# ANSSI-FR/libecc

Hardware: AMD Instinct MI355X
Metric: scalar-mults/sec (secp256r1, batch=2^20, variable base, affine out, bit-exact vs CPU) (higher is better)
Workload: dtype u32 (29-bit limbs, v_mad_u64_u32 integer MAD, u64 accumulators)

## Files before the change

libecc_amd/build.py:

```python
import os
import subprocess
import sys

HERE = os.path.dirname(os.path.abspath(__file__))
CSRC = os.path.join(HERE, "csrc")
LIBDIR = os.path.join(HERE, "lib")
LIB = os.path.join(LIBDIR, "libecc_amd.so")
SOURCES = ["ecamd_kernels.hip", "ecamd_p256_kernel.hip", "ecamd_hash.hip", "ecamd_host.cpp", "ecamd_multi.cpp"]
DEPS = ["ecamd_madchain.h", "ecamd_field.h", "ecamd_point.h", "ecamd_u29.h", "ecamd_p256.h", "ecamd_u29g.h", "ecamd_jacg.h",
        "ecamd_internal.h", "ecamd_lattice.h", "ecamd_randmod.h", "ecamd_recover.h", "ecamd_recover_kernels.h",
        "ecamd_sigfam.h", "ecamd_sigfam_kernels.h", "ecamd_sighash.h", "ecamd_sighash_kernels.h",
        "ecamd_curve_table.inc"]
HOST_DEPS = [os.path.join("..", "..", "include", "libecc_amd.h")]
HIPCC = os.environ.get("HIPCC", "/opt/rocm/bin/hipcc")
FLAGS = ["--offload-arch=gfx950", "-O3", "-std=c++17", "-fPIC", "-Wall", "-Wno-unused-function",
         "-Wno-bitwise-instead-of-logical", "-DU29_ASM_MAD"]


def _stale(target, inputs):
    if not os.path.exists(target):
        return True
    t = os.path.getmtime(target)
    return any(os.path.getmtime(i) > t for i in inputs)


G29_SIZES = [192, 224, 255, 256, 320, 384, 448, 511, 512, 521]


def _jobs():
    jobs = [(src, os.path.splitext(src)[0] + ".o", []) for src in SOURCES]
    jobs += [("ecamd_g29_kernel.hip", f"ecamd_g29_{pb}.o", [f"-DG29_PB={pb}"] + (["-DG29_WAVES=2"] if pb in (511, 512, 521) else []))
             for pb in G29_SIZES]
    jobs.append(("ecamd_g29_kernel.hip", "ecamd_g29_521m.o", ["-DG29_PB=521", "-DG29_M521P", "-DG29_WAVES=2"]))
    jobs.append(("ecamd_g29_kernel.hip", "ecamd_g29_255c.o", ["-DG29_PB=255", "-DG29_P25519", "-DG29_WAVES=3"]))
    jobs.append(("ecamd_g29_kernel.hip", "ecamd_g29_256k.o", ["-DG29_PB=256", "-DG29_K256", "-DG29_WAVES=3"]))
    jobs.append(("ecamd_g29_kernel.hip", "ecamd_g29_448g.o", ["-DG29_PB=448", "-DG29_P448"]))
    jobs.append(("ecamd_g29_kernel.hip", "ecamd_g29_384n.o", ["-DG29_PB=384", "-DG29_P384S"]))
    jobs.append(("ecamd_g29_kernel.hip", "ecamd_g29_224s.o", ["-DG29_PB=224", "-DG29_P224S"]))
    jobs.append(("ecamd_g29_kernel.hip", "ecamd_g29_192s.o", ["-DG29_PB=192", "-DG29_P192S"]))
    jobs.append(("ecamd_g29_kernel.hip", "ecamd_g29_dispatch.o", ["-DG29_DISPATCH"]))
    return jobs


def build(force=False, verbose=False):
    from concurrent.futures import ThreadPoolExecutor
    os.makedirs(LIBDIR, exist_ok=True)
    deps = [os.path.join(CSRC, d) for d in DEPS]
    hdeps = [os.path.join(CSRC, d) for d in HOST_DEPS]
    todo, objs = [], []
    for src, obj, extra in _jobs():
        spath, opath = os.path.join(CSRC, src), os.path.join(LIBDIR, obj)
        objs.append(opath)
        cmd = [HIPCC] + FLAGS + extra + ["-x", "hip", "-c", spath, "-o", opath]
        try:
            same_cmd = open(opath + ".cmd").read() == " ".join(cmd)
        except OSError:
            same_cmd = False
        if force or not same_cmd or _stale(opath, [spath] + deps + (hdeps if src.endswith(".cpp") else [])):
            todo.append(cmd)

    def run(cmd):
        if verbose:
            print(" ".join(cmd))
        subprocess.check_call(cmd)
        if "-c" in cmd:
            with open(cmd[-1] + ".cmd", "w") as f:
                f.write(" ".join(cmd))

    with ThreadPoolExecutor(max_workers=max(1, min(8, os.cpu_count() or 1))) as ex:
        list(ex.map(run, todo))
    if force or _stale(LIB, objs):
        run([HIPCC, "--offload-arch=gfx950", "-shared", "-fPIC", "-o", LIB] + objs + ["-ldl", "-lpthread"])
    return LIB


if __name__ == "__main__":
    print(build(force="--force" in sys.argv, verbose=True))
```

libecc_amd/csrc/ecamd_host.cpp:

```cpp
#include <hip/hip_runtime.h>
#include <stdint.h>
#include <string.h>
#include <strings.h>
#include <stdio.h>
#include <stdlib.h>
#include <string>
#include <vector>
#include <functional>
#include <mutex>
#include <sys/random.h>

#include "../../include/libecc_amd.h"
#include "ecamd_internal.h"
#include "ecamd_sighash.h"

static thread_local std::string g_err;
static int fail(const std::string &m)
{
	g_err = m;
	return -1;
}
#define HIPCHK(expr) \
	do { \
		hipError_t e_ = (expr); \
// ... 103 lines not shown
	big_trim(r);
	return r;
}
static Big big_mod(const Big &a, const Big &m)
{
	Big r(1, 0);
	for (int bit = big_bitlen(a) - 1; bit >= 0; bit--) {
		Big t(r.size() + 1, 0);
		for (size_t i = 0; i < r.size(); i++) {
			t[i] |= r[i] << 1;
			t[i + 1] |= r[i] >> 31;
		}
		t[0] |= (a[(size_t)bit / 32] >> (bit % 32)) & 1u;
		big_trim(t);
		r = (big_cmp(t, m) >= 0) ? big_sub(t, m) : t;
	}
	return r;
}
static Big big_pow2(int e)
{
	Big r((size_t)e / 32 + 1, 0);
	r[(size_t)e / 32] = 1u << (e % 32);
	return r;
}
static Big big_mulmod(const Big &a, const Big &b, const Big &m) { return big_mod(big_mul(a, b), m); }
static Big big_powmod(const Big &a, const Big &e, const Big &m)
{
	Big r(1, 1), base = big_mod(a, m);
	for (int i = big_bitlen(e) - 1; i >= 0; i--) {
		r = big_mulmod(r, r, m);
		if ((e[(size_t)i / 32] >> (i % 32)) & 1u) {
			r = big_mulmod(r, base, m);
		}
	}
	return r;
}
static void big_store(uint32_t *dst, int nw, const Big &a)
{
	for (int i = 0; i < nw; i++) {
		dst[i] = (size_t)i < a.size() ? a[(size_t)i] : 0;
	}
}
static void big_to_be(uint8_t *dst, int len, const Big &a)
{
	for (int i = 0; i < len; i++) {
		int pos = len - 1 - i;
		dst[i] = ((size_t)pos / 4 < a.size()) ? (uint8_t)(a[(size_t)pos / 4] >> (8 * (pos % 4))) : 0;
	}
}

struct CurveRow {
	const char *name;
	int type;
	const char *p, *a, *b, *order, *gx, *gy, *q, *h;
};
static const CurveRow g_curve_rows[] = {
#include "ecamd_curve_table.inc"
};

#define ECAMD_NSTAGE 30
struct ecamd_ctx {
	int device;
	hipStream_t stream;
	uint32_t max_chunk;
	uint32_t *tbl;
	size_t tbl_bytes;
	uint32_t *tbl_fast;
	size_t tbl_fast_bytes;
	uint8_t *prep_scratch;
	size_t prep_scratch_bytes;
	uint8_t *stage[ECAMD_NSTAGE];
	size_t stage_bytes[ECAMD_NSTAGE];
	hipEvent_t busy;
	hipStream_t last_stream;
	bool inflight;
	hipStream_t copy_stream;
	hipEvent_t in_ready[2];
	hipStream_t side_stream;
	hipEvent_t side_fork, side_done, side_mid, side_aux;
	hipEvent_t side_hi, side_red;
	hipStream_t side2_stream;
	hipEvent_t side2_fork, side2_done;
	bool side2_ok;
	bool side_ok;
	uint32_t host_chunk;
	uint32_t host_first_min;
	ecamd_host_ready_fn ready_fn = nullptr;
	void *ready_arg = nullptr;
	uint8_t *hbuf[2][6];
	size_t hbuf_bytes[2][6];
	uint32_t comb_min_batch;
	bool secret_scalars;
	int eddsa_msm;
	uint32_t msm_min, msm_k;
	uint8_t *msm;
	size_t msm_bytes;
	uint8_t msm_seed_bytes[32];
	bool msm_seed_valid;
	bool timing;
	hipEvent_t ev[ECAMD_NTIMED + 1];
	bool ev_valid;
	hipEvent_t ev_dom[2];
	bool ev_dom_valid;
	std::mutex mu;
};

struct ecamd_curve {
	ecamd_ctx *ctx;
	int nw;
	int slot;
	int qslot;
	int curve_type;
	int qnw;
	int clen;
	int qlen;
	int pbits, qbits;
	Big p, a, b, order, gx, gy, q;
	uint8_t *d_gen;
	uint32_t cofactor;
	int ed_state;
	const char *ed_err;
	EcamdEdDecodeArgs ed_tmpl;
	uint32_t ed_cof_dbl;
	int ed448_state;
	const char *ed448_err;
	EcamdEd448DecodeArgs ed448_tmpl;
	uint8_t ed448_c4[56];
	uint32_t ed_2d[9];
	uint32_t ed_Bx[9], ed_By[9];
	int xdh_state;
	const char *xdh_err;
	EcamdXdhPrepArgs xdh_tmpl;
	uint32_t xdh_A3[17];
	uint8_t xdh_cof;
	int sqrt_state;
	EcamdYfromXArgs sqrt_tmpl;
	bool is_p256;
	int gslot;
	int gpslot;
	int gqslot;
	int gflavour;
	uint32_t *d_comb4;
	bool comb4_off;
	uint32_t *d_gtab;
	uint32_t *d_comb;
	bool comb_off;
	uint32_t *d_edcomb;
	bool edcomb_off;
	uint32_t qdig[9];
};

static const int k_widths[] = {6, 7, 8, 10, 12, 14, 16, 17};

static int pick_nw(int pbits)
{
	for (int w : k_widths) {
		if (32 * w >= pbits) {
			return w;
		}
	}
	return 0;
}

extern "C" int ecamd_device_count(void)
{
	int n = 0;
// ... 27 lines not shown
		if (getenv("ECAMD_NO_COMB") != nullptr) {
			c->comb_min_batch = 0;
		}
	}
	c->tbl = nullptr;
	c->tbl_bytes = 0;
	c->tbl_fast = nullptr;
	c->tbl_fast_bytes = 0;
	for (int i = 0; i < ECAMD_NSTAGE; i++) {
		c->stage[i] = nullptr;
		c->stage_bytes[i] = 0;
	}
	c->prep_scratch = nullptr;
	c->prep_scratch_bytes = 0;
	c->last_stream = nullptr;
	c->inflight = false;
	if (hipEventCreateWithFlags(&c->busy, hipEventDisableTiming) != hipSuccess) {
		delete c;
		return fail("ecamd_ctx_create: hipEventCreate failed");
	}
	c->timing = false;
	c->secret_scalars = false;
	c->eddsa_msm = 1;
	c->msm_min = 1u << 17;
	c->msm_k = 0;
	{
		const char *e = getenv("ECAMD_MSM_MIN");
		if (e) {
			c->msm_min = (uint32_t)strtoul(e, nullptr, 10);
		}
		e = getenv("ECAMD_MSM_K");
		if (e) {
			c->msm_k = (uint32_t)strtoul(e, nullptr, 10);
		}
	}
	c->msm = nullptr;
	c->msm_bytes = 0;
	c->msm_seed_valid = false;
	c->ev_valid = false;
	c->ev_dom_valid = false;
	for (int i = 0; i <= ECAMD_NTIMED; i++) {
		if (hipEventCreate(&c->ev[i]) != hipSuccess) {
			delete c;
			return fail("ecamd_ctx_create: hipEventCreate failed");
		}
	}
	if (hipEventCreate(&c->ev_dom[0]) != hipSuccess || hipEventCreate(&c->ev_dom[1]) != hipSuccess) {
		delete c;
		return fail("ecamd_ctx_create: hipEventCreate failed");
	}
	memset(c->hbuf, 0, sizeof(c->hbuf));
	memset(c->hbuf_bytes, 0, sizeof(c->hbuf_bytes));
	{
		const char *e = getenv("ECAMD_HOST_CHUNK");
		c->host_chunk = e ? (uint32_t)strtoul(e, nullptr, 10) : (1u << 19);
		if (c->host_chunk == 0) {
			c->host_chunk = 1u << 19;
		}
		e = getenv("ECAMD_HOST_RAMP_MIN");
		c->host_first_min = e ? (uint32_t)strtoul(e, nullptr, 10) : (1u << 16);
		if (c->host_first_min == 0) {
			c->host_first_min = 1u << 16;
		}
	}
	if (hipStreamCreateWithFlags(&c->copy_stream, hipStreamNonBlocking) != hipSuccess ||
	    hipEventCreateWithFlags(&c->in_ready[0], hipEventDisableTiming) != hipSuccess ||
	    hipEventCreateWithFlags(&c->in_ready[1], hipEventDisableTiming) != hipSuccess) {
		delete c;
		return fail("ecamd_ctx_create: copy stream creation failed");
	}
	if (hipStreamCreateWithFlags(&c->stream, hipStreamNonBlocking) != hipSuccess) {
		delete c;
		return fail("ecamd_ctx_create: hipStreamCreate failed");
	}
	if (hipStreamCreateWithFlags(&c->side_stream, hipStreamNonBlocking) != hipSuccess ||
	    hipEventCreateWithFlags(&c->side_fork, hipEventDisableTiming) != hipSuccess ||
	    hipEventCreateWithFlags(&c->side_done, hipEventDisableTiming) != hipSuccess ||
	    hipEventCreateWithFlags(&c->side_mid, hipEventDisableTiming) != hipSuccess ||
	    hipEventCreateWithFlags(&c->side_aux, hipEventDisableTiming) != hipSuccess ||
	    hipEventCreateWithFlags(&c->side_hi, hipEventDisableTiming) != hipSuccess ||
	    hipEventCreateWithFlags(&c->side_red, hipEventDisableTiming) != hipSuccess ||
	    hipStreamCreateWithFlags(&c->side2_stream, hipStreamNonBlocking) != hipSuccess ||
	    hipEventCreateWithFlags(&c->side2_fork, hipEventDisableTiming) != hipSuccess ||
	    hipEventCreateWithFlags(&c->side2_done, hipEventDisableTiming) != hipSuccess) {
		delete c;
		return fail("ecamd_ctx_create: side stream creation failed");
	}
	c->side_ok = getenv("ECAMD_NO_SIDE_STREAM") == nullptr;
	c->side2_ok = c->side_ok;
	*out = c;
	return 0;
}

extern "C" void ecamd_ctx_destroy(ecamd_ctx *c)
{
	if (!c) {
		return;
	}
	(void)hipSetDevice(c->device);
	(void)hipStreamSynchronize(c->stream);
	if (c->tbl) {
		(void)hipFree(c->tbl);
	}
	if (c->tbl_fast) {
		(void)hipFree(c->tbl_fast);
	}
	if (c->msm) {
		(void)hipFree(c->msm);
	}
	for (int i = 0; i < ECAMD_NSTAGE; i++) {
		if (c->stage[i]) {
			(void)hipFree(c->stage[i]);
		}
	}
	if (c->prep_scratch) {
		(void)hipFree(c->prep_scratch);
	}
	for (int i = 0; i <= ECAMD_NTIMED; i++) {
		(void)hipEventDestroy(c->ev[i]);
	}
	(void)hipEventDestroy(c->ev_dom[0]);
	(void)hipEventDestroy(c->ev_dom[1]);
	(void)hipStreamDestroy(c->stream);
	(void)hipStreamDestroy(c->copy_stream);
	(void)hipStreamSynchronize(c->side_stream);
	(void)hipStreamDestroy(c->side_stream);
	(void)hipEventDestroy(c->side_fork);
	(void)hipEventDestroy(c->side_done);
	(void)hipEventDestroy(c->side_mid);
	(void)hipEventDestroy(c->side_aux);
	(void)hipEventDestroy(c->side_hi);
	(void)hipEventDestroy(c->side_red);
	(void)hipStreamSynchronize(c->side2_stream);
	(void)hipStreamDestroy(c->side2_stream);
	(void)hipEventDestroy(c->side2_fork);
	(void)hipEventDestroy(c->side2_done);
	(void)hipEventDestroy(c->in_ready[0]);
	(void)hipEventDestroy(c->in_ready[1]);
	(void)hipEventDestroy(c->busy);
	for (int b = 0; b < 2; b++) {
		for (int k = 0; k < 6; k++) {
			if (c->hbuf[b][k]) {
				(void)hipFree(c->hbuf[b][k]);
			}
		}
	}
	delete c;
}

extern "C" int ecamd_ctx_set_max_chunk(ecamd_ctx *c, uint32_t max_items)
{
	if (!c || max_items == 0) {
		return fail("ecamd_ctx_set_max_chunk: bad argument");
	}
	c->max_chunk = max_items;
	return 0;
}

extern "C" int ecamd_ctx_set_eddsa_msm(ecamd_ctx *c, int mode, uint32_t min_items, uint32_t items_per_lane)
{
	if (!c || mode < 0 || mode > 2 || items_per_lane > 64) {
		return fail("ecamd_ctx_set_eddsa_msm: bad argument");
	}
	std::lock_guard<std::mutex> lk(c->mu);
	c->eddsa_msm = mode;
	if (min_items) {
		c->msm_min = min_items;
	}
	c->msm_k = items_per_lane;
	return 0;
}

extern "C" int ecamd_ctx_set_msm_seed(ecamd_ctx *c, const uint8_t seed[32])
{
	if (!c || !seed) {
		return fail("ecamd_ctx_set_msm_seed: bad argument");
	}
	std::lock_guard<std::mutex> lk(c->mu);
	memcpy(c->msm_seed_bytes, seed, 32);
	c->msm_seed_valid = true;
	return 0;
}

extern "C" int ecamd_ctx_discard_msm_seed(ecamd_ctx *c)
{
	if (!c) {
		return fail("ecamd_ctx_discard_msm_seed: NULL context");
	}
	std::lock_guard<std::mutex> lk(c->mu);
	if (c->msm_seed_valid) {
		memset(c->msm_seed_bytes, 0, sizeof(c->msm_seed_bytes));
		c->msm_seed_valid = false;
	}
	return 0;
}

extern "C" int ecamd_ctx_set_secret_scalars(ecamd_ctx *c, int on)
{
	if (!c) {
		return fail("ecamd_ctx_set_secret_scalars: NULL context");
	}
	std::lock_guard<std::mutex> lk(c->mu);
	c->secret_scalars = on != 0;
	return 0;
}

extern "C" int ecamd_ctx_enable_kernel_timing(ecamd_ctx *c, int on)
{
	if (!c) {
		return fail("ecamd_ctx_enable_kernel_timing: NULL context");
	}
	std::lock_guard<std::mutex> lk(c->mu);
	c->timing = on != 0;
	c->ev_valid = false;
	c->ev_dom_valid = false;
	return 0;
}

extern "C" int ecamd_ctx_kernel_times(ecamd_ctx *c, double *ms, int n)
// ... 907 lines not shown
	const bool secret = ctx->secret_scalars;
	const bool fast256 = cv->is_p256 && slen <= 68;
	const bool fastg = !fast256 && cv->gslot >= 0 && slen <= ecamd_g29_max_slen(cv->pbits);
	const bool comb_ok = !secret && (cv->is_p256 ? slen <= 32 : slen <= ecamd_g29_comb_max_slen(cv->pbits));
	const bool fast = !redo_only && (fast256 || fastg);
	if (fast && !d_points && comb_ok) {
		maybe_build_comb(ctx, const_cast<ecamd_curve *>(cv), n);
	}
	if (fast && fastg && !d_points && secret && n >= 64) {
		maybe_build_comb4(ctx, const_cast<ecamd_curve *>(cv));
	}
	{
		uint8_t *t = (uint8_t *)ctx->tbl;
		const int rc = ensure(&t, &ctx->tbl_bytes, tbl_bytes_for(cv, stride));
		ctx->tbl = (uint32_t *)t;
		if (rc) {
			return -1;
		}
	}
	if (fast) {
		uint8_t *t = (uint8_t *)ctx->tbl_fast;
		const size_t per_item = fast256 ? P256_SCRATCH_PER_ITEM
						: ((size_t)ecamd_g29_table_words(cv->pbits, cv->gflavour) + ecamd_g29_affine_words(cv->pbits, cv->gflavour)) * 4;
		const int rc = ensure(&t, &ctx->tbl_fast_bytes, (size_t)stride * per_item);
		ctx->tbl_fast = (uint32_t *)t;
		if (rc) {
			return -1;
		}
	}
	for (uint32_t off = 0; off < n; off += chunk) {
		const uint32_t m = (n - off) < chunk ? (n - off) : chunk;
		EcamdSmulArgs A;
		A.scalars = d_scalars + (size_t)off * sstride;
		A.sstride = sstride;
		A.pstride = d_points ? 2u * (uint32_t)cv->clen : 0u;
		A.points = d_points ? d_points + (size_t)off * 2 * cv->clen : cv->d_gen;
		A.out = d_out + (size_t)off * 2 * cv->clen;
		A.status = d_status + off;
		A.tbl = ctx->tbl;
		A.n = m;
		A.slen = slen;
		A.clen = (uint32_t)cv->clen;
		A.stride = stride;
		A.slot = cv->slot;
		A.only_redo = redo_only ? 1 : 0;
		A.lut = nullptr;
		A.lut_kind = 0;
		A.stg = nullptr;
		A.masked = secret ? 1 : 0;
		A.scalars2 = nullptr;
		A.s2len = 0;
		if (d_scalars2) {
			if (!fastg || !d_points || !cv->d_comb) {
				return fail("internal: fused double-scalar loop requested without its preconditions");
			}
			EcamdSmulArgs Fa = A;
			Fa.tbl = ctx->tbl_fast;
			Fa.stg = ctx->tbl_fast + (size_t)stride * (size_t)ecamd_g29_table_words(cv->pbits, cv->gflavour);
			Fa.lut = cv->d_comb;
			Fa.lut_kind = 2u;
			Fa.scalars2 = d_scalars2 + (size_t)off * slen;
			Fa.s2len = slen;
			Fa.masked = 0;
			hipEvent_t *ev = (ctx->timing && off == 0) ? ctx->ev : nullptr;
			HIPCHK(ecamd_launch_smul_g29(cv->pbits, cv->gslot, Fa, s, ev, cv->gflavour));
			ctx->ev_valid = ctx->ev_valid || (ev != nullptr);
			continue;
		}
		if (fast) {
			EcamdSmulArgs Fa = A;
			Fa.tbl = ctx->tbl_fast;
			Fa.stg = ctx->tbl_fast + (size_t)stride * (fast256 ? (size_t)(P256_TAB_BYTES / 4) : (size_t)ecamd_g29_table_words(cv->pbits, cv->gflavour));
			if (!d_points) {
				const bool use_comb = cv->d_comb && comb_ok;
				Fa.lut = use_comb ? cv->d_comb : (fast256 ? cv->d_gtab : nullptr);
				Fa.lut_kind = use_comb ? 1u : 0u;
				if (secret && cv->d_comb4 && (fast256 ? slen <= 32 : slen <= 4 * (uint32_t)((cv->pbits + 31) / 32))) {
					Fa.lut = cv->d_comb4;
					Fa.lut_kind = 3u;
				}
			}
			hipEvent_t *ev = (ctx->timing && off == 0) ? ctx->ev : nullptr;
			if (fast256) {
				HIPCHK(ecamd_launch_smul_p256(Fa, s, ev));
			} else {
				HIPCHK(ecamd_launch_smul_g29(cv->pbits, cv->gslot, Fa, s, ev, cv->gflavour));
			}
			ctx->ev_valid = ctx->ev_valid || (ev != nullptr);
			A.only_redo = 1;
		}
		HIPCHK(ecamd_launch_smul(cv->nw, A, s));
	}
	return 0;
}

struct HostArr {
	const uint8_t *in;
	uint8_t *out;
	size_t stride;
};

template <class Core>
static int host_pipeline(ecamd_ctx *ctx, int pbits, uint32_t n, const std::vector<HostArr> &arrs, Core core, uint32_t even_chunk = 0)
{
	const uint32_t chunk = even_chunk && even_chunk < ctx->host_chunk ? (n < even_chunk ? n : even_chunk) : (n < ctx->host_chunk ? n : ctx->host_chunk);
	const size_t na = arrs.size();
	if (na > 6) {
		return fail("internal: too many host arrays");
	}
	static const bool no_ramp = getenv("ECAMD_NO_HOST_RAMP") != nullptr;
	std::vector<uint32_t> sched;
	{
		uint32_t left = n;
		if (const char *e = getenv("ECAMD_HOST_SCHEDULE")) {
			while (*e && left) {
				uint32_t v = (uint32_t)strtoul(e, nullptr, 10);
				v = v < 1 ? 1 : (v > left ? left : v);
				sched.push_back(v);
				left -= v;
				e = strchr(e, ',');
				if (!e) {
					break;
				}
				e++;
			}
		} else if (even_chunk && n > chunk) {
			const uint32_t m = ctx->host_first_min < chunk ? ctx->host_first_min : chunk;
			if (m < chunk && left > m) {
				sched.push_back(m);
				left -= m;
			}
		} else if (n > chunk && !no_ramp && pbits <= 256) {
			for (uint32_t m = ctx->host_first_min < chunk ? ctx->host_first_min : chunk; m < chunk && left > m + m; m += m) {
				sched.push_back(m);
				left -= m;
			}
		} else if (n > chunk && !no_ramp) {
			const uint32_t m = chunk / 8 < ctx->host_first_min ? ctx->host_first_min : chunk / 8;
			if (m < chunk) {
				sched.push_back(m);
				left -= m;
			}
		}
		while (left) {
			const uint32_t m = (left <= chunk + chunk / 4) ? left : chunk;
			sched.push_back(m);
			left -= m;
		}
	}
	uint32_t largest = 0;
	for (uint32_t m : sched) {
		largest = m > largest ? m : largest;
	}
	const int nbuf = sched.size() > 1 ? 2 : 1;
	for (int b = 0; b < nbuf; b++) {
		for (size_t k = 0; k < na; k++) {
			if (ensure(&ctx->hbuf[b][k], &ctx->hbuf_bytes[b][k], (size_t)largest * arrs[k].stride)) {
				return -1;
			}
		}
	}
	hipStream_t cs = ctx->copy_stream, s = ctx->stream;
	StreamScope scope(ctx, s);
	auto copy_in = [&](uint32_t off, uint32_t m, int b) -> int {
		if (ctx->ready_fn) {
			ctx->ready_fn(ctx->ready_arg, off, m);
		}
// ... 4617 lines not shown
```

libecc_amd/csrc/ecamd_internal.h:

```cpp
#pragma once
#include <stdlib.h>
#include <hip/hip_runtime.h>
#include <stdint.h>

#define ECAMD_WINDOW 4
#define ECAMD_TBL_ENTRIES (1 << ECAMD_WINDOW)
#define ECAMD_STATUS_TAB 0xFC
#define ECAMD_STATUS_JAC 0xFD
#define ECAMD_STATUS_REDO 0xFE
#define ECAMD_MAX_SLOTS_HOST 16
#define P256_TAB_BYTES 512u
#define P256_STG_QUADS 70u

struct EcamdSmulArgs {
	const uint8_t *scalars;
	const uint8_t *points;
	uint8_t *out;
	uint8_t *status;
	uint32_t *tbl;
	uint32_t *stg;
	uint32_t n, slen, clen, pstride, stride;
	uint32_t sstride;
	int slot;
	int only_redo;
// ... 53 lines not shown
	uint8_t *result;
	uint32_t n, clen, qlen, jmax;
	uint32_t q[17];
	int slot;
	const uint8_t *only;
};
struct EcamdEcdsaSignArgs {
	const uint8_t *privs, *nonces, *digests;
	const uint8_t *kG, *stkG;
	uint8_t *sigs, *status;
	uint32_t n, clen, qlen, hlen, qbits, jmax;
	int qslot;
};
hipError_t ecamd_launch_ecdsa_sign(int nw, const EcamdEcdsaSignArgs &a, hipStream_t s);
hipError_t ecamd_launch_ecdsa_prep(int nw, const EcamdEcdsaPrepArgs &a, hipStream_t s);
hipError_t ecamd_launch_ecdsa_fin(int nw, const EcamdEcdsaFinArgs &a, hipStream_t s);

struct EcamdSigPrepArgs {
	EcamdEcdsaPrepArgs p;
	uint8_t *target;
	int alg;
};
struct EcamdSigSignArgs {
	EcamdEcdsaSignArgs a;
	int alg;
};
hipError_t ecamd_launch_sig_prep(int nw, const EcamdSigPrepArgs &a, hipStream_t s);
hipError_t ecamd_launch_sig_sign(int nw, const EcamdSigSignArgs &a, hipStream_t s);

struct EcamdRecoverPrepArgs {
	const uint8_t *sigs;
	const uint8_t *digests;
	uint8_t *u, *v;
	uint8_t *x;
	uint8_t *flags;
	uint32_t n, qlen, clen, hlen, qbits;
	int qslot;
	uint8_t p_be[72];
};
struct EcamdRecoverPointArgs {
	const uint8_t *x, *y1;
	const uint8_t *flags, *yst;
	uint8_t *R;
	uint32_t n, clen;
};
struct EcamdRecoverFinArgs {
	const uint8_t *A, *stA;
	const uint8_t *B, *stB;
	const uint8_t *flags;
	const uint8_t *yst;
	uint8_t *out1, *out2;
	uint8_t *st1, *st2;
	uint32_t n, clen;
	int slot;
};
hipError_t ecamd_launch_recover_prep(int qnw, const EcamdRecoverPrepArgs &a, hipStream_t s);
hipError_t ecamd_launch_recover_point(const EcamdRecoverPointArgs &a, hipStream_t s);
hipError_t ecamd_launch_recover_fin(int nw, const EcamdRecoverFinArgs &a, hipStream_t s);
hipError_t ecamd_launch_recover_redo(int nw, const EcamdRecoverFinArgs &a, hipStream_t s);

struct EcamdHsigArgs {
	const uint8_t *sigs;
	const uint8_t *inputs;
	const uint8_t *privs, *nonces;
	uint8_t *u, *v;
	uint8_t *flags;
	const uint8_t *W, *stW;
	uint8_t *slots;
	const uint8_t *dg;
	uint8_t *out;
	uint8_t *status;
	uint32_t n, qlen, clen, hsize, sstride;
	int qslot, alg, sign;
};
hipError_t ecamd_launch_hsig_prep(int qnw, const EcamdHsigArgs &a, hipStream_t s);
hipError_t ecamd_launch_hsig_fill(const EcamdHsigArgs &a, hipStream_t s);
hipError_t ecamd_launch_hsig_cmp(const EcamdHsigArgs &a, hipStream_t s);
hipError_t ecamd_launch_hsig_sign(int qnw, const EcamdHsigArgs &a, hipStream_t s);

int ecamd_nw_supported(int nw);
hipError_t ecamd_upload_curve(int nw, int slot, const void *curvek, size_t bytes);
hipError_t ecamd_launch_smul(int nw, const EcamdSmulArgs &a, hipStream_t s);
#define ECAMD_NTIMED 5
hipError_t ecamd_launch_smul_p256(const EcamdSmulArgs &a, hipStream_t s, hipEvent_t *ev);
hipError_t ecamd_launch_verify_p256(const EcamdSmulArgs &pubkeys, const uint8_t *u1, const uint8_t *u2, const uint8_t *sigs,
				    const uint8_t *flags, const uint32_t *gtbl, int gtbl_is_comb, const uint32_t *qdigits,
				    uint8_t *result, hipStream_t s, hipEvent_t *dom = nullptr, hipEvent_t scalars_ready = nullptr);
hipError_t ecamd_launch_comb_build_p256(const uint8_t *points, uint32_t n, uint32_t *table, hipStream_t s);
struct EcamdXdhPrepArgs {
	const uint8_t *k, *u;
	uint8_t *scalars;
	uint8_t *points;
	uint8_t *flags;
	uint32_t n, len, ebits, mode;
	uint32_t cof_dbl;
	uint32_t e[17];
	uint32_t A[17], A3[17], sm1[17];
	uint32_t g_A[16], g_A3[16], g_sm1[16];
	int slot;
};
struct EcamdXdhFinArgs {
	const uint8_t *pts;
	const uint8_t *stk;
	const uint8_t *flags;
	uint8_t *out;
	uint8_t *status;
	uint32_t n, len;
	uint32_t A3[17];
	int slot;
};
hipError_t ecamd_launch_xdh_prep(int nw, const EcamdXdhPrepArgs &a, hipStream_t s);
hipError_t ecamd_launch_xdh_fin(int nw, const EcamdXdhFinArgs &a, hipStream_t s);

struct EcamdEdDecodeArgs {
	const uint8_t *encA;
	const uint8_t *encR;
	uint32_t strideA, strideR;
	uint8_t *pointsA, *pointsR;
	uint8_t *flagsA, *flagsR;
	uint32_t n, len, cof_dbl;
	uint32_t a[17], d[17], sm1[17], alpha[17], A3[17];
	uint32_t g_d[9], g_sm1[9], g_alpha[9], g_A3[9];
	uint32_t *edA;
	uint32_t *edR;
	int slot;
};
hipError_t ecamd_launch_ed_decode_ed_c25519(const EcamdEdDecodeArgs &a, int gslot, hipStream_t s);
struct EcamdEdSmulArgs {
	const uint32_t *edA;
	const uint8_t *scalars;
	const uint8_t *flags;
	uint32_t *tbl;
	uint32_t *rec;
	uint8_t *out, *status;
	uint32_t n;
	uint32_t g_2d[9], g_alpha[9], g_A3[9];
	const uint32_t *edR;
	uint8_t *flagsR;
	uint8_t *outR;
};
#define ECAMD_EDT_ITEM_WORDS 320
#define ECAMD_EDR_REC_WORDS 28
struct EcamdEdTailConsts {
	uint32_t g_2d[9], g_alpha[9], g_A3[9];
};
#define ECAMD_EDC_ENT_WORDS 32
#define ECAMD_EDC_ENTRIES (16u * 32768u + 1u)
struct EcamdEdSmul2Args {
	const uint32_t *edA, *edR;
	const uint8_t *flagsA, *flagsR, *flagsS;
	const uint32_t *uv;
	const uint8_t *meta;
	uint32_t *tbl;
	uint32_t *rec;
	uint32_t n;
	uint32_t g_2d[9];
};
struct EcamdEdTailArgs {
	const uint32_t *rec;
	const uint32_t *edR;
	const uint8_t *flagsA, *flagsR, *flagsS;
	const uint8_t *S_be;
	const uint8_t *sp_be;
	const uint8_t *meta;
	const uint32_t *comb;
	uint8_t *result;
	uint32_t n, cof_dbl;
// ... 348 lines not shown
```

libecc_amd/csrc/ecamd_p256_kernel.hip:

```cpp
#include <hip/hip_runtime.h>
#include "ecamd_p256.h"
#include "ecamd_internal.h"

using namespace p256;

typedef uint8_t u8;

#define TBL_WORDS_PER_ENTRY 40
#define TBL_ENTRIES 8
#define TAB_ENT_WORDS 16
#define TAB_ITEM_WORDS (TBL_ENTRIES * TAB_ENT_WORDS)
#define STG_ENT_QUADS 10
#define STG_ITEM_QUADS (7 * STG_ENT_QUADS)
static_assert(TAB_ITEM_WORDS * 4 <= P256_TAB_BYTES && STG_ITEM_QUADS <= P256_STG_QUADS, "scratch exceeds the host's per-item sizing");
#ifndef FIN_K
#define FIN_K 8
#endif
#ifndef AFF_K
#define AFF_K 8
#endif
static inline int p256_items_per_inversion(uint32_t n, int kmax)
{
	const int k = n >= (1u << 19) ? 8 : (n >= (1u << 17) ? 4 : 2);
	return k < kmax ? k : kmax;
}

static __device__ __forceinline__ void load_be256(const u8 *src, u32 *w)
{
	if ((((uintptr_t)src) & 15) == 0) {
		const uint4 a = *(const uint4 *)src, b = *(const uint4 *)(src + 16);
		w[7] = __builtin_bswap32(a.x);
		w[6] = __builtin_bswap32(a.y);
		w[5] = __builtin_bswap32(a.z);
		w[4] = __builtin_bswap32(a.w);
		w[3] = __builtin_bswap32(b.x);
		w[2] = __builtin_bswap32(b.y);
		w[1] = __builtin_bswap32(b.z);
		w[0] = __builtin_bswap32(b.w);
	} else {
#pragma unroll
		for (int i = 0; i < 8; i++) {
			const u8 *q = src + 4 * (7 - i);
			w[i] = ((u32)q[0] << 24) | ((u32)q[1] << 16) | ((u32)q[2] << 8) | (u32)q[3];
		}
	}
}

static __device__ __forceinline__ void store_be256(u8 *dst, const u32 *w)
{
	if ((((uintptr_t)dst) & 15) == 0) {
		uint4 a, b;
		a.x = __builtin_bswap32(w[7]);
		a.y = __builtin_bswap32(w[6]);
		a.z = __builtin_bswap32(w[5]);
		a.w = __builtin_bswap32(w[4]);
		b.x = __builtin_bswap32(w[3]);
		b.y = __builtin_bswap32(w[2]);
		b.z = __builtin_bswap32(w[1]);
		b.w = __builtin_bswap32(w[0]);
		*(uint4 *)dst = a;
		*(uint4 *)(dst + 16) = b;
	} else {
#pragma unroll
		for (int i = 0; i < 8; i++) {
			u8 *q = dst + 4 * (7 - i);
			q[0] = (u8)(w[i] >> 24);
			q[1] = (u8)(w[i] >> 16);
			q[2] = (u8)(w[i] >> 8);
			q[3] = (u8)w[i];
		}
	}
}

static __device__ __forceinline__ bool lt_p(const u32 *w)
{
	constexpr u32 pw[8] = {0xffffffffu, 0xffffffffu, 0xffffffffu, 0x00000000u, 0x00000000u, 0x00000000u, 0x00000001u, 0xffffffffu};
	u32 borrow = 0;
#pragma unroll
	for (int i = 0; i < 8; i++) {
		const uint64_t x = (uint64_t)w[i] - pw[i] - borrow;
		borrow = (u32)(x >> 63);
	}
	return borrow != 0;
}

// ... 953 lines not shown
		return;
	}
	if (inf) {
		A.result[i] = 1;
		return;
	}
	u32 rw[8];
	load_be256(A.sigs + (size_t)i * 64, rw);
	const Fcanon r2c = constant<Fcanon>(K::R2), onec = constant<Fcanon>(K::ONE);
	const auto z2 = sqr(acc.Z);
	const Fcanon rd = from_words(rw);
	const auto t1 = mul(mul(rd, r2c), z2);
	bool acc_ok = is_zero_mulout(mul(carry(sub<1, 1>(t1, acc.X)), onec));
	{
		u32 sdg[9];
		u32 cy = 0;
#pragma unroll
		for (int w = 0; w < 9; w++) {
			const u32 x = rd.l[w] + A.qd[w] + cy;
			cy = (w < 8) ? (x >> 29) : 0u;
			sdg[w] = (w < 8) ? (x & MASK) : x;
		}
		u32 bw = 0;
#pragma unroll
		for (int w = 0; w < 9; w++) {
			bw = (sdg[w] - P256::P[w] - bw) >> 31;
		}
		Fcanon rq;
#pragma unroll
		for (int w = 0; w < 9; w++) {
			rq.l[w] = bw ? sdg[w] : 0u;
		}
		const auto t2 = mul(mul(rq, r2c), z2);
		acc_ok = acc_ok | ((bw != 0) & is_zero_mulout(mul(carry(sub<1, 1>(t2, acc.X)), onec)));
	}
	A.result[i] = acc_ok ? 0 : 1;
}

hipError_t ecamd_launch_verify_p256(const EcamdSmulArgs &pubkeys, const uint8_t *u1, const uint8_t *u2, const uint8_t *sigs,
				    const uint8_t *flags, const uint32_t *gtbl, int gtbl_is_comb, const uint32_t *qdigits,
				    uint8_t *result, hipStream_t s, hipEvent_t *dom, hipEvent_t scalars_ready)
{
	if (pubkeys.n == 0) {
		return scalars_ready ? hipStreamWaitEvent(s, scalars_ready, 0) : hipSuccess;
	}
	const dim3 grid((pubkeys.n + 63) / 64), block(64);
	const uint32_t ak = (uint32_t)p256_items_per_inversion(pubkeys.n, AFF_K);
	const uint32_t athreads = (((pubkeys.n + ak - 1) / ak) + 63u) & ~63u;
	hipLaunchKernelGGL(k_p256_table, grid, block, 0, s, pubkeys);
	hipLaunchKernelGGL(k_p256_affine, dim3((athreads + 63) / 64), block, 0, s, pubkeys, athreads, (int)ak);
	P256VerifyArgs V;
	V.u1 = u1;
	V.u2 = u2;
	V.sigs = sigs;
	V.flags = flags;
	V.status = pubkeys.status;
	V.qtbl = pubkeys.tbl;
	V.gtbl = gtbl;
	V.result = result;
	V.n = pubkeys.n;
	for (int w = 0; w < 9; w++) {
		V.qd[w] = qdigits[w];
	}
	if (scalars_ready) {
		const hipError_t e = hipStreamWaitEvent(s, scalars_ready, 0);
		if (e != hipSuccess) {
			return e;
		}
	}
	if (dom) {
		(void)hipEventRecord(dom[0], s);
	}
	if (gtbl_is_comb) {
		hipLaunchKernelGGL(k_p256_verify_loop<true>, grid, block, 0, s, V);
	} else {
		hipLaunchKernelGGL(k_p256_verify_loop<false>, grid, block, 0, s, V);
	}
	if (dom) {
		(void)hipEventRecord(dom[1], s);
	}
	return hipGetLastError();
}

hipError_t ecamd_launch_smul_p256(const EcamdSmulArgs &a, hipStream_t s, hipEvent_t *ev)
{
	if (a.n == 0) {
		return hipSuccess;
	}
	const dim3 grid((a.n + 63) / 64), block(64);
	const uint32_t fk = (uint32_t)p256_items_per_inversion(a.n, FIN_K);
	const uint32_t nthreads = (((a.n + fk - 1) / fk) + 63u) & ~63u;
	const dim3 fgrid((nthreads + 63) / 64);
#define P256_MARK(i) do { if (ev) (void)hipEventRecord(ev[i], s); } while (0)
	P256_MARK(0);
	if (a.lut) {
		(void)hipMemsetAsync(a.status, ECAMD_STATUS_TAB, a.n, s);
		P256_MARK(1);
	} else {
		const uint32_t ak = (uint32_t)p256_items_per_inversion(a.n, AFF_K);
		const uint32_t athreads = (((a.n + ak - 1) / ak) + 63u) & ~63u;
		if (P256_ODD_WINDOWS) {
			hipLaunchKernelGGL(k_p256_table_odd, grid, block, 0, s, a);
			P256_MARK(1);
			hipLaunchKernelGGL(k_p256_affine_coz, dim3((athreads + 63) / 64), block, 0, s, a, athreads, (int)ak);
		} else {
			hipLaunchKernelGGL(k_p256_table, grid, block, 0, s, a);
			P256_MARK(1);
			hipLaunchKernelGGL(k_p256_affine, dim3((athreads + 63) / 64), block, 0, s, a, athreads, (int)ak);
		}
	}
	P256_MARK(2);
	if (!a.lut && P256_ODD_WINDOWS) {
		if (a.masked) {
			if (a.slen <= 32) {
				hipLaunchKernelGGL((k_p256_loop_odd<8, true>), grid, block, 0, s, a);
			} else {
				hipLaunchKernelGGL((k_p256_loop_odd<17, true>), grid, block, 0, s, a);
			}
		} else if (a.slen <= 32) {
			hipLaunchKernelGGL((k_p256_loop_odd<8, false>), grid, block, 0, s, a);
		} else {
			hipLaunchKernelGGL((k_p256_loop_odd<17, false>), grid, block, 0, s, a);
		}
	} else if (a.lut && a.lut_kind == 1) {
		hipLaunchKernelGGL(k_p256_comb, grid, block, 0, s, a);
	} else if (a.lut && a.lut_kind == 3) {
		hipLaunchKernelGGL(k_p256_comb4m, grid, block, 0, s, a);
	} else {
		if (a.masked) {
			if (a.slen <= 32) {
				hipLaunchKernelGGL((k_p256_loop<8, true>), grid, block, 0, s, a);
			} else {
				hipLaunchKernelGGL((k_p256_loop<17, true>), grid, block, 0, s, a);
			}
		} else if (a.slen <= 32) {
			hipLaunchKernelGGL((k_p256_loop<8, false>), grid, block, 0, s, a);
		} else {
			hipLaunchKernelGGL((k_p256_loop<17, false>), grid, block, 0, s, a);
		}
	}
	P256_MARK(3);
	hipLaunchKernelGGL(k_p256_finalize, fgrid, block, 0, s, a, nthreads, (int)fk);
	P256_MARK(4);
	return hipGetLastError();
}

hipError_t ecamd_launch_comb_build_p256(const uint8_t *points, uint32_t n, uint32_t *table, hipStream_t s)
{
	if (n == 0) {
		return hipSuccess;
	}
	hipLaunchKernelGGL(k_p256_comb_build, dim3((n + 63) / 64), dim3(64), 0, s, points, n, table);
	return hipGetLastError();
}
```

Baseline: 75.72 million.

## Split P256 scalar-mult batch into two chunks overlapped on side stream

Adds a planner that splits the p256 variable-base batch into a head of whole occupancy rounds and a remainder tail. The tail chain (table, affine, loop, finalize) runs on the side stream while the head runs on the main stream, joined by events. The aim is to let the partial last wave of one chunk overlap with the other chunk's work instead of leaving CUs idle between stages. Inversion batch sizes are still derived from the full batch size. The split only happens when the batch is not an exact multiple of the round size, and it adds extra launches and event synchronisation.

Measured after the change: 72.31 million. -4.5%, worse.

```diff
diff --git a/libecc_amd/build.py b/libecc_amd/build.py
--- a/libecc_amd/build.py
+++ b/libecc_amd/build.py
@@ -8,7 +8,7 @@
 LIB = os.path.join(LIBDIR, "libecc_amd.so")
 SOURCES = ["ecamd_kernels.hip", "ecamd_p256_kernel.hip", "ecamd_hash.hip", "ecamd_host.cpp", "ecamd_multi.cpp"]
 DEPS = ["ecamd_madchain.h", "ecamd_field.h", "ecamd_point.h", "ecamd_u29.h", "ecamd_p256.h", "ecamd_u29g.h", "ecamd_jacg.h",
-        "ecamd_internal.h", "ecamd_lattice.h", "ecamd_randmod.h", "ecamd_recover.h", "ecamd_recover_kernels.h",
+        "ecamd_internal.h", "ecamd_p256_plan.h", "ecamd_lattice.h", "ecamd_randmod.h", "ecamd_recover.h", "ecamd_recover_kernels.h",
         "ecamd_sigfam.h", "ecamd_sigfam_kernels.h", "ecamd_sighash.h", "ecamd_sighash_kernels.h",
         "ecamd_curve_table.inc"]
 HOST_DEPS = [os.path.join("..", "..", "include", "libecc_amd.h")]
diff --git a/libecc_amd/csrc/ecamd_host.cpp b/libecc_amd/csrc/ecamd_host.cpp
--- a/libecc_amd/csrc/ecamd_host.cpp
+++ b/libecc_amd/csrc/ecamd_host.cpp
@@ -209,6 +209,8 @@
 	hipStream_t side2_stream;
 	hipEvent_t side2_fork, side2_done;
 	bool side2_ok;
+	hipEvent_t p256_fork, p256_join;
+	uint32_t cus;
 	bool side_ok;
 	uint32_t host_chunk;
 	uint32_t host_first_min;
@@ -402,9 +404,19 @@
 	    hipEventCreateWithFlags(&c->side_red, hipEventDisableTiming) != hipSuccess ||
 	    hipStreamCreateWithFlags(&c->side2_stream, hipStreamNonBlocking) != hipSuccess ||
 	    hipEventCreateWithFlags(&c->side2_fork, hipEventDisableTiming) != hipSuccess ||
-	    hipEventCreateWithFlags(&c->side2_done, hipEventDisableTiming) != hipSuccess) {
+	    hipEventCreateWithFlags(&c->side2_done, hipEventDisableTiming) != hipSuccess ||
+	    hipEventCreateWithFlags(&c->p256_fork, hipEventDisableTiming) != hipSuccess ||
+	    hipEventCreateWithFlags(&c->p256_join, hipEventDisableTiming) != hipSuccess) {
 		delete c;
 		return fail("ecamd_ctx_create: side stream creation failed");
+	}
+	{
+		int cus = 0;
+		if (hipDeviceGetAttribute(&cus, hipDeviceAttributeMultiprocessorCount, device) != hipSuccess || cus < 0) {
+			(void)hipGetLastError();
+			cus = 0;
+		}
+		c->cus = (uint32_t)cus;
 	}
 	c->side_ok = getenv("ECAMD_NO_SIDE_STREAM") == nullptr;
 	c->side2_ok = c->side_ok;
@@ -455,6 +467,8 @@
 	(void)hipStreamDestroy(c->side2_stream);
 	(void)hipEventDestroy(c->side2_fork);
 	(void)hipEventDestroy(c->side2_done);
+	(void)hipEventDestroy(c->p256_fork);
+	(void)hipEventDestroy(c->p256_join);
 	(void)hipEventDestroy(c->in_ready[0]);
 	(void)hipEventDestroy(c->in_ready[1]);
 	(void)hipEventDestroy(c->busy);
@@ -1528,7 +1542,10 @@
 			}
 			hipEvent_t *ev = (ctx->timing && off == 0) ? ctx->ev : nullptr;
 			if (fast256) {
-				HIPCHK(ecamd_launch_smul_p256(Fa, s, ev));
+				const char *pe = getenv("ECAMD_P256_PIPELINE");
+				const EcamdP256Pipe pipe = {ctx->side_stream, ctx->p256_fork, ctx->p256_join, ctx->cus};
+				const bool split = ctx->side_ok && !(pe && atoi(pe) == 0) && s != ctx->side_stream;
+				HIPCHK(ecamd_launch_smul_p256(Fa, s, ev, split ? &pipe : nullptr));
 			} else {
 				HIPCHK(ecamd_launch_smul_g29(cv->pbits, cv->gslot, Fa, s, ev, cv->gflavour));
 			}
diff --git a/libecc_amd/csrc/ecamd_internal.h b/libecc_amd/csrc/ecamd_internal.h
--- a/libecc_amd/csrc/ecamd_internal.h
+++ b/libecc_amd/csrc/ecamd_internal.h
@@ -159,7 +159,12 @@
 hipError_t ecamd_upload_curve(int nw, int slot, const void *curvek, size_t bytes);
 hipError_t ecamd_launch_smul(int nw, const EcamdSmulArgs &a, hipStream_t s);
 #define ECAMD_NTIMED 5
-hipError_t ecamd_launch_smul_p256(const EcamdSmulArgs &a, hipStream_t s, hipEvent_t *ev);
+struct EcamdP256Pipe {
+	hipStream_t side;
+	hipEvent_t fork, join;
+	uint32_t cus;
+};
+hipError_t ecamd_launch_smul_p256(const EcamdSmulArgs &a, hipStream_t s, hipEvent_t *ev, const EcamdP256Pipe *pipe = nullptr);
 hipError_t ecamd_launch_verify_p256(const EcamdSmulArgs &pubkeys, const uint8_t *u1, const uint8_t *u2, const uint8_t *sigs,
 				    const uint8_t *flags, const uint32_t *gtbl, int gtbl_is_comb, const uint32_t *qdigits,
 				    uint8_t *result, hipStream_t s, hipEvent_t *dom = nullptr, hipEvent_t scalars_ready = nullptr);
diff --git a/libecc_amd/csrc/ecamd_p256_kernel.hip b/libecc_amd/csrc/ecamd_p256_kernel.hip
--- a/libecc_amd/csrc/ecamd_p256_kernel.hip
+++ b/libecc_amd/csrc/ecamd_p256_kernel.hip
@@ -1,6 +1,7 @@
 #include <hip/hip_runtime.h>
 #include "ecamd_p256.h"
 #include "ecamd_internal.h"
+#include "ecamd_p256_plan.h"
 
 using namespace p256;
 
@@ -1120,22 +1121,25 @@
 	return hipGetLastError();
 }
 
-hipError_t ecamd_launch_smul_p256(const EcamdSmulArgs &a, hipStream_t s, hipEvent_t *ev)
-{
-	if (a.n == 0) {
-		return hipSuccess;
-	}
+#ifndef P256_PIPELINE
+#define P256_PIPELINE 1
+#endif
+
+static void p256_enqueue_chain(const EcamdSmulArgs &a, uint32_t n_batch, hipStream_t s, hipEvent_t *ev, bool mark0, hipEvent_t join)
+{
 	const dim3 grid((a.n + 63) / 64), block(64);
-	const uint32_t fk = (uint32_t)p256_items_per_inversion(a.n, FIN_K);
+	const uint32_t fk = (uint32_t)p256_items_per_inversion(n_batch, FIN_K);
 	const uint32_t nthreads = (((a.n + fk - 1) / fk) + 63u) & ~63u;
 	const dim3 fgrid((nthreads + 63) / 64);
 #define P256_MARK(i) do { if (ev) (void)hipEventRecord(ev[i], s); } while (0)
-	P256_MARK(0);
+	if (mark0) {
+		P256_MARK(0);
+	}
 	if (a.lut) {
 		(void)hipMemsetAsync(a.status, ECAMD_STATUS_TAB, a.n, s);
 		P256_MARK(1);
 	} else {
-		const uint32_t ak = (uint32_t)p256_items_per_inversion(a.n, AFF_K);
+		const uint32_t ak = (uint32_t)p256_items_per_inversion(n_batch, AFF_K);
 		const uint32_t athreads = (((a.n + ak - 1) / ak) + 63u) & ~63u;
 		if (P256_ODD_WINDOWS) {
 			hipLaunchKernelGGL(k_p256_table_odd, grid, block, 0, s, a);
@@ -1179,7 +1183,58 @@
 	}
 	P256_MARK(3);
 	hipLaunchKernelGGL(k_p256_finalize, fgrid, block, 0, s, a, nthreads, (int)fk);
+	if (join) {
+		(void)hipStreamWaitEvent(s, join, 0);
+	}
 	P256_MARK(4);
+#undef P256_MARK
+}
+
+static_assert(P256_TAB_BYTES % 64u == 0, "a chunk's table records must stay on their 64-byte alignment");
+static EcamdSmulArgs p256_chunk_args(const EcamdSmulArgs &a, const P256Chunk &c)
+{
+	EcamdSmulArgs b = a;
+	b.scalars = a.scalars + (size_t)c.off * a.sstride;
+	b.points = a.points + (size_t)c.off * a.pstride;
+	b.out = a.out + (size_t)c.off * 2 * a.clen;
+	b.status = a.status + c.off;
+	b.tbl = a.tbl + (size_t)c.off * (P256_TAB_BYTES / 4);
+	b.stg = a.stg + (size_t)c.off * (P256_STG_QUADS * 4);
+	b.n = c.n;
+	return b;
+}
+
+hipError_t ecamd_launch_smul_p256(const EcamdSmulArgs &a, hipStream_t s, hipEvent_t *ev, const EcamdP256Pipe *pipe)
+{
+	if (a.n == 0) {
+		return hipSuccess;
+	}
+	P256Chunk ch[2];
+	int nch = 1;
+	if (P256_PIPELINE && P256_ODD_WINDOWS && pipe && !a.lut) {
+		nch = p256_plan_chunks(a.n, pipe->cus * 4u * (uint32_t)P256_WAVES * 64u, ch);
+	}
+	if (nch == 1) {
+		p256_enqueue_chain(a, a.n, s, ev, true, nullptr);
+		return hipGetLastError();
+	}
+	if (ev) {
+		(void)hipEventRecord(ev[0], s);
+	}
+	hipError_t e = hipEventRecord(pipe->fork, s);
+	if (e == hipSuccess) {
+		e = hipStreamWaitEvent(pipe->side, pipe->fork, 0);
+	}
+	if (e != hipSuccess) {
+		return e;
+	}
+	p256_enqueue_chain(p256_chunk_args(a, ch[0]), a.n, pipe->side, nullptr, false, nullptr);
+	e = hipEventRecord(pipe->join, pipe->side);
+	if (e != hipSuccess) {
+		(void)hipStreamSynchronize(pipe->side);
+		return e;
+	}
+	p256_enqueue_chain(p256_chunk_args(a, ch[1]), a.n, s, ev, false, pipe->join);
 	return hipGetLastError();
 }
 
diff --git a/libecc_amd/csrc/ecamd_p256_plan.h b/libecc_amd/csrc/ecamd_p256_plan.h
--- /dev/null
+++ b/libecc_amd/csrc/ecamd_p256_plan.h
@@ -0,0 +1,41 @@
+#pragma once
+#include <stdint.h>
+
+#define P256_CHUNK_ALIGN 512u
+static_assert(P256_CHUNK_ALIGN % 64u == 0, "a chunk must start on a staging block (64 items)");
+static_assert(P256_CHUNK_ALIGN % (8u * 64u) == 0, "a chunk must start on a whole wave of eight-item lanes");
+
+struct P256Chunk {
+	uint32_t off, n;
+	int side;
+};
+
+#ifndef P256_PIPELINE_MIN_ROUNDS
+#define P256_PIPELINE_MIN_ROUNDS 2u
+#endif
+static inline uint32_t p256_pipeline_min_items(uint32_t round)
+{
+	return P256_PIPELINE_MIN_ROUNDS * round;
+}
+
+static inline int p256_plan_chunks(uint32_t n, uint32_t round, P256Chunk out[2])
+{
+	out[0].off = 0;
+	out[0].n = n;
+	out[0].side = 0;
+	if (round == 0 || n < p256_pipeline_min_items(round)) {
+		return 1;
+	}
+	const uint32_t head = (n / round) * round / P256_CHUNK_ALIGN * P256_CHUNK_ALIGN;
+	const uint32_t rest = n - head;
+	if (head == 0 || rest < round / 16u || rest == 0) {
+		return 1;
+	}
+	out[0].off = head;
+	out[0].n = rest;
+	out[0].side = 1;
+	out[1].off = 0;
+	out[1].n = head;
+	out[1].side = 0;
+	return 2;
+}
```
